# mhsitu/welding_robot

Measured on AMD Instinct MI355X. Metric: acs_generations_per_sec, higher is better.
Workload: dtype f32

## Files before the change

welding_robot_amd/csrc/acs_converged.hpp:

```cpp
#pragma once

#define WA_CONV_CHECK_WAVES 4
#define WA_CONV_ADV_WAVES 4
#define WA_CONV_THREADS ((WA_CONV_CHECK_WAVES + WA_CONV_ADV_WAVES) * 64)
#define WA_CONV_BLOCKS 64
#define WA_CONV_BLOCKS_MAX 256
#define WA_CONV_MAX_WINDOW 64
#define WA_CONV_NODE_CAP 1024
#define WA_CONV_NODE_LDS 128
#define WA_CONV_SNAP 14

struct WaConvHdr {
    uint32_t rem;
    uint32_t ticket;
    int32_t pending;
    int32_t carried;
    unsigned long long whole, cut, gens;
    int32_t end;
    int32_t pad1_;
    unsigned long long walks;
    unsigned long long pad2_;
};
static_assert(WA_CONV_SNAP == 14, "wa_table_rows strides the owed records by 14 floats");
static_assert(sizeof(WaConvHdr) == 64, "the snapshots start 64 bytes into the block");

__device__ __forceinline__ WaConvHdr *wa_conv_hdr(const WaAcsDev &D, int32_t slot) { return reinterpret_cast<WaConvHdr *>(D.conv + (int64_t)slot * D.conv_stride); }
__device__ __forceinline__ float *wa_conv_snap(const WaAcsDev &D, int32_t slot, int32_t t)
{
    return reinterpret_cast<float *>(D.conv + (int64_t)slot * D.conv_stride + sizeof(WaConvHdr)) + (int64_t)t * D.conv_nodes * WA_CONV_SNAP;
}
__device__ __forceinline__ int32_t wa_conv_pending(const WaAcsDev &D, int32_t slot) { return wa_conv_hdr(D, slot)->pending; }
__device__ __forceinline__ bool wa_conv_carried(const WaAcsDev &D, int32_t slot) { return wa_conv_hdr(D, slot)->carried != 0; }
__device__ __forceinline__ bool wa_conv_carried_at(const WaAcsDev &D, int32_t slot, int32_t gen)
{
    if (!D.conv) return false;
    const WaConvHdr *h = wa_conv_hdr(D, slot);
    return h->carried != 0 && h->end == gen && D.ctl[slot].spec_until == gen;
}
__device__ __forceinline__ void wa_conv_count_walk(const WaAcsDev &D, int32_t slot) { wa_conv_hdr(D, slot)->walks += 1; }
__device__ __forceinline__ const float *wa_conv_owed_records(const WaAcsDev &D, int32_t slot) { return wa_conv_snap(D, slot, wa_conv_pending(D, slot) - 1); }
#define WA_CONV_CARRIED 0x80u

__device__ __forceinline__ void wa_conv_flush_rows(const WaAcsDev &D, int32_t slot, int32_t first, int32_t step, bool rows_only)
{
    const int32_t blen = D.ctl[slot].best_len, j = wa_conv_pending(D, slot);
    if (j < 1) return;
    const float *snap = wa_conv_snap(D, slot, j - 1);
    const int32_t *bpath = D.bestpath + (int64_t)slot * D.path_cap;
    float *pher = D.pher + (int64_t)slot * D.pher_stride;
    float *T = D.rtab + (int64_t)slot * D.path_cap * 8;
    for (int32_t x = first; x < blen * WA_CONV_SNAP; x += step) {
        const int32_t i = x / WA_CONV_SNAP, q = x - i * WA_CONV_SNAP;
        const float v = snap[x];
        if (q < 6) { if (!rows_only) pher[(int64_t)(bpath[i] & (int32_t)WA_ID_MASK) * 6 + q] = v; }
        else T[(int64_t)i * 8 + (q - 6)] = v;
    }
}

__device__ __forceinline__ void wa_conv_ctl_step(WaSlotCtl &c, const WaRun &R, int32_t gen)
{
    const int32_t lane = threadIdx.x & 63, o = lane + 1;
    const int32_t colony = c.colony[gen & 1];
    const float lambda = c.lambda[gen & 1], Q = c.Q[gen & 1], bestL = c.bestL;
    const bool ok = lane < colony && !(bestL == INFINITY || (float)o > lambda - 1);
    const unsigned long long dep = __ballot(ok);
    const int32_t n_dep = dep ? 64 - (int32_t)__clzll((long long)dep) : 0;
    if (lane == 0) {
        c.dep_lambda = lambda;
        c.dep_Q = Q;
        c.dep_bestL = bestL;
        c.n_dep = n_dep;
        c.gen = gen + 1;
        c.rep_mask = n_dep >= 64 ? ~0ULL : (1ULL << n_dep) - 1ULL;
        c.clean[(gen + 1) & 1] = c.clean[gen & 1] * R.rho;
        wa_next_params(c, R, (gen + 1) & 1);
    }
}

__device__ __forceinline__ void wa_conv_report(uint32_t *verdict, int32_t slot, uint32_t seq, int32_t j, bool carried = false)
{
    if (!verdict) return;
    if (j > 0) {
        __threadfence_system();
        __hip_atomic_store(verdict + slot, (seq << 8) | (carried ? WA_CONV_CARRIED : 0u) | (uint32_t)j, __ATOMIC_RELEASE, __HIP_MEMORY_SCOPE_SYSTEM);
    } else __hip_atomic_store(verdict + slot, seq << 8, __ATOMIC_RELAXED, __HIP_MEMORY_SCOPE_SYSTEM);
}

__device__ __forceinline__ float wa_add_all_ranked(float p, bool on, float dep_lane, float bonus, int32_t n)
{
    n = __builtin_amdgcn_readfirstlane(n);
    const float t_lane = (int32_t)(threadIdx.x & 63) < n ? dep_lane + bonus : -0.f;
    float q = p;
    asm volatile("" : "+v"(q));
#pragma unroll
    for (int b0 = 0; b0 < 64; b0 += 8) {
        if (b0 >= n) break;
        float t[8];
#pragma unroll
        for (int j = 0; j < 8; j++) t[j] = __int_as_float(__builtin_amdgcn_readlane(__float_as_int(t_lane), b0 + j));
#pragma unroll
        for (int j = 0; j < 8; j++) q = q + t[j];
    }
    return on ? q : p;
}

__host__ __device__ inline int32_t wa_conv_share(int32_t nodes, int32_t blocks) { return (nodes + blocks - 1) / blocks; }

struct WaConvShared {
    WaSlotCtl tab[WA_CONV_MAX_WINDOW + 1];
    unsigned long long key[WA_CONV_MAX_WINDOW + 1];
    int32_t bad[WA_CONV_MAX_WINDOW + 1];
    int32_t run;
    int32_t last, j, carried;
};
__host__ __device__ inline size_t wa_conv_lds_bytes(int32_t conv_nodes, int32_t blocks)
{
    return (size_t)wa_conv_share(conv_nodes, blocks) * WA_CONV_NODE_LDS + sizeof(WaConvShared);
}

__global__ __launch_bounds__(WA_CONV_THREADS) void k_converged_run(WaAcsDev D, WaRun R, int32_t gen0, int32_t W, uint32_t *verdict, uint32_t seq, int32_t judge)
{
    extern __shared__ __attribute__((aligned(16))) float wa_conv_lds[];
    const int32_t slot = blockIdx.y, blk = blockIdx.x, nblk = gridDim.x, tid = threadIdx.x, lane = tid & 63, wave = tid >> 6;
    WaSlotCtl *ctl = &D.ctl[slot];
    WaConvHdr *hdr = wa_conv_hdr(D, slot);
    const float bestL = ctl->bestL;
    const int32_t blen = ctl->best_len;
    bool off = bestL == INFINITY || blen < 2 || blen > D.conv_nodes || blen > WA_CONV_NODE_CAP || W < 1 || W > WA_CONV_MAX_WINDOW;
    if (D.pool_n) {
        const WaStrag sg = wa_strag_of(D, slot);
        off = off || sg.pool_n[0] != 0 || sg.pool_n[1] != 0;
    }
    if (off) {
        if (blk == 0 && tid == 0) wa_conv_report(verdict, slot, seq, 0);
        return;
    }
    const int32_t cap = wa_conv_share(D.conv_nodes, nblk);
    const int32_t m = wa_conv_share(blen, nblk), n0 = blk * m;
    const int32_t mine = blen - n0 < 0 ? 0 : blen - n0 < m ? blen - n0 : m;
    const int32_t last = blen - 1;
    const int32_t ndec = (n0 + mine < last ? n0 + mine : last) - n0;
    float *s_row = wa_conv_lds;
    float *s_rec = wa_conv_lds + cap * 16;
    WaConvShared &S = *reinterpret_cast<WaConvShared *>(wa_conv_lds + cap * 32);
    {
        const int32_t *bpath = D.bestpath + (int64_t)slot * D.path_cap + n0;
        const uint8_t *btabu = D.besttabu + (int64_t)slot * D.path_cap + n0;
        const float *pher = D.pher + (int64_t)slot * D.pher_stride;
        const float *heur = D.heur + (int64_t)ctl->heur_slot * D.pher_stride;
        const float *T = D.rtab + ((int64_t)slot * D.path_cap + n0) * 8;
        for (int32_t x = tid; x < mine * 16; x += WA_CONV_THREADS) {
            const int32_t i = x >> 4, q = x & 15;
            const int64_t v = bpath[i] & (int32_t)WA_ID_MASK;
            s_rec[x] = q < 6 ? pher[v * 6 + q] : q < 12 ? heur[v * 6 + q - 6] : q == 12 ? __uint_as_float((uint32_t)btabu[i]) : 0.f;
        }
        for (int32_t x = tid; x < mine * 8; x += WA_CONV_THREADS) {
            const float v = T[x];
            s_row[x] = v;
            if ((x & 7) == 7) s_row[cap * 8 + x] = v;
        }
    }
    if (wave == 0) {
        if (lane == 0) S.tab[0] = *ctl;
        int32_t run = 0;
        for (; run < W; run++) {
            const int32_t gen = gen0 + run;
            const int32_t colony = S.tab[run].colony[gen & 1];
            if (!(colony >= 1 && colony <= D.max_colony)) break;
            if (lane == 0) S.tab[run + 1] = S.tab[run];
            wa_conv_ctl_step(S.tab[run + 1], R, gen);
        }
        if (lane == 0) S.run = run;
    } else if (wave == 1) {
        for (int32_t t = lane; t <= W; t += 64) {
            S.key[t] = wa_ctr_key(R.seed, ctl->stream, (uint32_t)(gen0 + t));
            S.bad[t] = 0;
        }
    }
    __syncthreads();
    const int32_t run = S.run;
    int32_t my_t = mine > 0 ? run : W;
    for (int32_t t = 0; t < run && mine > 0; t++) {
        const int32_t gen = gen0 + t;
        const int32_t colony = S.tab[t].colony[gen & 1];
        const float *row = s_row + (t & 1) * cap * 8;
        if (wave < WA_CONV_CHECK_WAVES) {
            const uint64_t genkey = S.key[t];
            for (int32_t a = tid; a < colony; a += WA_CONV_CHECK_WAVES * 64) {
                const uint64_t antkey = wa_ctr_antkey(genkey, (uint32_t)a);
                bool bad = false;
                for (int32_t n = 0; n < ndec; n++) {
                    const float4 *r4 = reinterpret_cast<const float4 *>(row + n * 8);
                    const float4 ca = r4[0], cb = r4[1];
                    const uint32_t h = wa_replay_hits(ca, cb, (int32_t)wa_ctr_draw(antkey, (uint32_t)(n0 + n)));
                    const int pick = h ? 31 - __clz((int)h) : -1;
                    bad = bad || pick != __float_as_int(cb.w);
                }
                if (bad) S.bad[t] = 1;
            }
        } else {
            const WaSlotCtl &c = S.tab[t + 1];
            const int32_t n_dep = c.n_dep;
            const float lambda = c.dep_lambda, Q = c.dep_Q;
            const bool okl = lane < colony && lane < n_dep;
            const float dep_lane = okl ? (lambda - (float)(lane + 1)) * Q / bestL : 0.f;
            const float bonus_on = wa_uniform(1.f * lambda * Q / bestL);
            float *nrow = s_row + ((t + 1) & 1) * cap * 8;
            float *snap = wa_conv_snap(D, slot, t) + (int64_t)n0 * WA_CONV_SNAP;
            const int32_t k2 = lane & 15, kk = k2 < 6 ? k2 : 5;
            for (int32_t i = (wave - WA_CONV_CHECK_WAVES) * 4 + (lane >> 4); __any(i < mine); i += WA_CONV_ADV_WAVES * 4) {
                const bool live = i < mine;
                const int32_t ii = live ? i : 0;
                const int32_t nk = __float_as_int(row[ii * 8 + 7]);
                float p = s_rec[ii * 16 + kk] * R.rho;
                const float h = s_rec[ii * 16 + 6 + kk];
                const uint32_t bt = __float_as_uint(s_rec[ii * 16 + 12]);
                p = wa_add_all_ranked(p, live && k2 == nk, dep_lane, bonus_on, n_dep);
                float thr, tot;
                wa_row_values(R, p, h, k2, bt, thr, tot);
                if (!live) continue;
                float *sn = snap + i * WA_CONV_SNAP;
                if (k2 < 6) {
                    s_rec[i * 16 + k2] = p;
                    nrow[i * 8 + k2] = thr;
                    sn[k2] = p;
                    sn[6 + k2] = thr;
                }
                if (k2 == 5) { nrow[i * 8 + 6] = tot; sn[12] = tot; }
                if (k2 == 0) sn[13] = __int_as_float(nk);
            }
        }
        __syncthreads();
        if (S.bad[t] != 0) { my_t = t; break; }
    }
    int32_t leaves = 1;
    if (judge && run == W && my_t == W) {
        const int32_t gen = gen0 + W;
        const int32_t colony = S.tab[W].colony[gen & 1];
        leaves = !(colony >= 1 && colony <= D.max_colony);
        if (!leaves && mine > 0) {
            if (wave < WA_CONV_CHECK_WAVES) {
                const float *row = s_row + (W & 1) * cap * 8;
                const uint64_t genkey = S.key[W];
                for (int32_t a = tid; a < colony; a += WA_CONV_CHECK_WAVES * 64) {
                    const uint64_t antkey = wa_ctr_antkey(genkey, (uint32_t)a);
                    bool bad = false;
                    for (int32_t n = 0; n < ndec; n++) {
                        const float4 *r4 = reinterpret_cast<const float4 *>(row + n * 8);
                        const float4 ca = r4[0], cb = r4[1];
                        const uint32_t h = wa_replay_hits(ca, cb, (int32_t)wa_ctr_draw(antkey, (uint32_t)(n0 + n)));
                        const int pick = h ? 31 - __clz((int)h) : -1;
                        bad = bad || pick != __float_as_int(cb.w);
                    }
                    if (bad) S.bad[W] = 1;
                }
            }
            __syncthreads();
            leaves = S.bad[W] != 0;
        }
    }
    if (tid == 0) {
        atomicMax(&hdr->rem, ((uint32_t)(W - my_t) << 1) | (uint32_t)leaves);
        __threadfence();
        const uint32_t tk = atomicAdd(&hdr->ticket, 1u);
        int32_t is_last = 0, j = 0, carried = 0;
        if (tk == (uint32_t)nblk - 1u) {
            __threadfence();
            is_last = 1;
            const uint32_t rem = atomicMax(&hdr->rem, 0u);
            j = W - (int32_t)(rem >> 1);
            carried = rem == 0u;
        }
        S.last = is_last;
        S.j = j;
        S.carried = carried;
    }
    __syncthreads();
    if (!S.last) return;
    const int32_t j = S.j;
    const bool carried = S.carried != 0;
    if (tid == 0) {
        hdr->rem = 0;
        hdr->ticket = 0;
        if (j > 0) {
            WaSlotCtl c = S.tab[j];
            c.spec_until = gen0 + j;
            *ctl = c;
            hdr->pending = j;
            hdr->carried = carried ? 1 : 0;
            hdr->end = gen0 + j;
            hdr->gens += (unsigned long long)j;
            if (j == W) hdr->whole += 1; else hdr->cut += 1;
        }
    }
    if (j > 0) {
        const int32_t colony = S.tab[j].colony[(gen0 + j - 1) & 1];
        const float lambda = S.tab[j].dep_lambda, Q = S.tab[j].dep_Q;
        for (int32_t r = tid; r < colony; r += WA_CONV_THREADS) {
            const int32_t o = r + 1;
            const bool ok = !(bestL == INFINITY || (float)o > lambda - 1);
            D.perm[(int64_t)slot * D.max_colony + r] = r;
            D.depA[(int64_t)slot * D.max_colony + r] = ok ? (lambda - (float)o) * Q / bestL : 0.f;
        }
        for (int32_t t = tid; t < j; t += WA_CONV_THREADS) {
            const int32_t gen = gen0 + t;
            if (gen >= D.trace_cap) continue;
            const int32_t col = S.tab[t].colony[gen & 1];
            const int64_t tr = (int64_t)slot * D.trace_cap + gen;
            D.trBest[tr] = bestL;
            D.trIter[tr] = bestL;
            D.trColony[tr] = col;
            D.trFinite[tr] = col;
            D.trSteps[tr] = (long long)col * (long long)(blen - 1);
        }
    }
    __syncthreads();
    if (tid == 0) wa_conv_report(verdict, slot, seq, j, carried);
}
```

welding_robot_amd/csrc/host_acs.inc:

```
static int acs_drain(wa_acs *s);
void wa_acs_default_params(wa_acs_params *p)
{
    if (!p) return;
    p->alpha = 1;
    p->beta = 0.6f;
    p->rho = 0.8f;
    p->pheromone_0 = 1.f;
    p->max_iteration = 150;
    p->predict = 10.f;
    p->fixed_colony = 0;
    p->rng_mode = WA_RNG_DEV;
    p->seed = 1;
}


static_assert(WA_PLAN_REF_SPEC_LEN == WA_REF_SPEC_LEN && WA_PLAN_REF_SUPER == WA_REF_SUPER && WA_PLAN_RESUME_MAX == WA_RESUME_MAX &&
              WA_PLAN_POOL_REC == WA_POOL_REC && WA_PLAN_ROW26 == WA_ROW26, "acs_plan.hpp and the kernels' headers disagree");
static WaPlanIn acs_plan_in(const wa_grid *grid, int32_t n_slots, int32_t max_colony, int64_t path_capacity, int32_t nb, bool lazy)
{
    int32_t fields0 = n_slots < 4 ? n_slots : 4;
    if (n_slots >= 32) fields0 = n_slots / 8 < 8 ? 8 : (n_slots / 8 > 24 ? 24 : n_slots / 8);
    return WaPlanIn{grid->d.n, grid->d.nxy, n_slots, max_colony, fields0, path_capacity, nb, lazy ? 1 : 0,
                    env_int("WA_MASK_U64", 0), env_int("WA_REPLAY", 1), env_int("WA_REF_SPEC", 1), env_int("WA_STRAGGLERS", 1), env_int("WA_STRAGGLER_SLOTS", 16),
                    (int64_t)sizeof(WaSlotCtl), (int64_t)sizeof(WaGlibcRand)};
// ... 40 lines not shown
    s->nb = nb;
    s->lazy = lazy;
    s->slot_buf.assign(n_slots, 0);
    s->lazy_mode.assign(n_slots, -1);
    s->lazy_p0.assign(n_slots, 0.f);
    if (nb == 6 && 24 * n >= (int64_t)1 << 31) {
        delete s;
        return fail(ctx, WA_ERR_ARG, "wa_acs_create: grids above 89,478,485 voxels (~447^3) are not supported");
    }
    if (nb == 26 && n > (int64_t)WaNbT<26>::IDM + 1) {
        delete s;
        return fail(ctx, WA_ERR_ARG, "wa_acs_create: 26-neighbour grids above 2^27 voxels (512^3) are not supported");
    }
    const WaAcsPlan &P = s->plan = wa_acs_plan(acs_plan_in(grid, n_slots, max_colony, path_capacity, nb, lazy));
    path_capacity = s->path_cap = P.cap;
    s->ref_spec = P.ref_spec;
    WaAcsDev &D = s->D;
    D.d = grid->d;
    D.cx = grid->cx; D.cy = grid->cy; D.cz = grid->cz; D.occ = grid->occ;
    D.nb = nb;
    D.max_colony = max_colony;
    D.pher_stride = P.pher_stride; D.path_cap = P.cap; D.vbits_words = P.vbits_words; D.vbits_rows = (int32_t)P.vbits_rows;
    D.guard_bytes = (int32_t)(P.guard * sizeof(float)); D.stamp_guard_bytes = (int32_t)(P.sguard * sizeof(uint32_t));
    int lg = 11;
    while ((1 << lg) < 64 * (grid->d.nx + grid->d.ny + grid->d.nz) && lg < 15) lg++;
    int id_bits = 1;
    while (((int64_t)1 << id_bits) < n) id_bits++;
    s->tab16_env = env_int("WA_TAB16", -1);
    s->id_bits = id_bits;
    D.tab16_kmul = 0;
    if (nb == 6 && id_bits <= 27 && s->tab16_env != 0) {
        uint32_t kb = (uint32_t)((double)((uint64_t)1 << id_bits) * 0.6180339887498949) | 1u;
        D.tab16_kmul = kb << (32 - id_bits);
    }
    {
        const int64_t blocks = (int64_t)n_slots * max_colony;
        const bool saturated = blocks > ctx->prop.multiProcessorCount;
        auto capacity = [&](int l) {
            const bool t16 = saturated && D.tab16_kmul != 0 && id_bits <= l + 12 && (s->tab16_env == 1 || id_bits <= 21);
            int64_t per_cu = 160 * 1024 / (((t16 ? 2 : 4) << l) + WA_WALK_LDS_EXTRA);
            if (per_cu > 16) per_cu = 16;
            return per_cu * ctx->prop.multiProcessorCount;
        };
        int floor_lg = 6;
        while (floor_lg < 15 && 3 * ((int64_t)1 << floor_lg) < 16 * (int64_t)(grid->d.nx + grid->d.ny + grid->d.nz)) floor_lg++;
        if (floor_lg < 10) floor_lg = 10;
        while (lg > floor_lg && capacity(lg) < blocks && capacity(lg - 1) > capacity(lg)) lg--;
        if (n_slots == 1 && !lazy && max_colony <= 256 && env_int("WA_STRAGGLERS", 1))
            while (lg > 12 && capacity(lg) < max_colony + WA_RESUME_MAX) lg--;
    }
    s->hash_log2 = env_int("WA_HASH_LOG2", lg);
    if (s->hash_log2 < 6) s->hash_log2 = 6;
    if (s->hash_log2 > 15) s->hash_log2 = 15;
    s->walk_asm = env_int("WA_WALK_ASM", 1) != 0;
    s->walk_warm = env_int("WA_WALK_WARM", -1);
    s->walk_direct = env_int("WA_WALK_DIRECT", -1);
    s->lds_pad = env_int("WA_WALK_LDS_PAD", 0);
    if (s->lds_pad < 0 || (sizeof(int32_t) << s->hash_log2) + (size_t)s->lds_pad > (sizeof(int32_t) << 15)) s->lds_pad = 0;
    {
        const int re = env_int("WA_REENTRY", 1);
        s->walk_flags = (s->walk_asm ? 1 : 0) | (re ? 2 : 0) | ((env_int("WA_REENTRY_STABLE", 16) & 127) << 24);
#ifdef WA_TEST_KNOBS
        s->walk_flags |= (re == 2 ? 4 : 0) | (env_int("WA_REENTRY_ANYWHERE", 0) ? 8 : 0) | ((env_int("WA_REENTRY_HOLD", 0) & 0xffff) << 8);
#endif
    }
    s->lazy_blocks_env = env_int("WA_LAZY_BLOCKS", 0);
    s->pipe_groups_env = env_int("WA_PIPE_GROUPS", 0);
    s->hw_queues = env_int("GPU_MAX_HW_QUEUES", 4);
    s->drain_ok = env_int("WA_STRAGGLER_DRAIN", 1) != 0;
    s->sweep_nt_env = env_int("WA_SWEEP_NT", -1);
    s->straggler_gens = env_int("WA_STRAGGLER_GENS", 64);
    s->conv_on = env_int("WA_CONVERGED_RUN", 1) != 0;
    s->conv_window = env_int("WA_CONVERGED_WINDOW", 32);
    if (s->conv_window > WA_CONV_MAX_WINDOW) s->conv_window = WA_CONV_MAX_WINDOW;
    if (s->conv_window < 1) s->conv_on = false;
    s->conv_nodes_env = env_int("WA_CONVERGED_NODES", 0);
    s->conv_blocks = env_int("WA_CONVERGED_BLOCKS", WA_CONV_BLOCKS);
    s->conv_blocks = s->conv_blocks < 1 ? 1 : s->conv_blocks > WA_CONV_BLOCKS_MAX ? WA_CONV_BLOCKS_MAX : s->conv_blocks;
    s->conv_readback = env_int("WA_CONVERGED_READBACK", 1) != 0;
    s->conv_wait_us = env_int("WA_CONVERGED_WAIT_US", 200000);
    s->conv_spec = env_int("WA_CONVERGED_SPECULATE", 1) != 0;
    s->conv_owed = env_int("WA_CONVERGED_OWED", 1) != 0;
    s->conv_cwalk = env_int("WA_CONVERGED_CARRIED_WALK", 1) != 0;
    s->prof_dispatch = env_int("WA_PROF_DISPATCH", 1) != 0;
    s->conv_enqueued.assign((size_t)n_slots, 0);
    {
        const int64_t n4 = (int64_t)nb * n / 4;
        int64_t blocks = n4 <= ((int64_t)8 << 20) ? 4096 : n4 / 555;
        if (blocks > 65536) blocks = 65536;
        s->evap_blocks = env_int("WA_EVAP_BLOCKS", (int)blocks);
    }
    hipError_t e = hipSuccess;
    const bool trace_create = env_int("WA_TRACE_CREATE", 0) != 0;
    const auto t_create0 = std::chrono::steady_clock::now();
    auto since0 = [&]() { return std::chrono::duration<double>(std::chrono::steady_clock::now() - t_create0).count(); };
    bool pools = P.pools;
    for (const WaPlanRow &r : P.rows) {
        if (e || (r.pool && !pools)) continue;
        if (&r == &P.rows[P.heur_row]) { e = (hipError_t)heur_pool_grow(s, &D, (int32_t)P.fields0); continue; }
        void *p = nullptr;
        const hipError_t re = ctx_alloc_bytes(ctx, &p, (size_t)P.bytes(r));
        if (re == hipSuccess) { s->blocks.push_back(WaBlock{&r, p}); continue; }
        if (!r.pool) { e = re; continue; }
        (void)hipGetLastError();
        pools = false;
        for (; s->blocks.back().row->pool; s->blocks.pop_back()) ctx_free(ctx, s->blocks.back().p);
    }
    size_t wired = 0;
    auto wire = [&](auto *&dst, const char *name, int64_t skip = 0) {
        using T = typename std::remove_reference<decltype(dst)>::type;
        for (const WaBlock &b : s->blocks)
            if (!strcmp(b.row->name, name)) { dst = static_cast<T>(b.p) + skip; wired++; }
    };
    uint32_t *ref_jump = nullptr;
    wire(s->pher_buf[0], "pher0", P.guard); wire(s->pher_buf[1], "pher1", P.guard); wire(D.heur, "heur", P.guard); wire(D.ltab, "ltab");
    wire(D.stamp, "stamp", P.sguard); wire(D.dirty_list, "dirty_list"); wire(D.dcount, "dcount");
    wire(D.mask8, "mask8"); wire(D.mask, "mask"); wire(D.bestmark, "bestmark"); wire(D.bestpath, "bestpath"); wire(D.bestpos, "bestpos"); wire(D.besttabu, "besttabu"); wire(D.rtab, "rtab");
    wire(D.paths, "paths"); wire(D.antL, "antL"); wire(D.antLen, "antLen"); wire(D.perm, "perm"); wire(D.depA, "depA"); wire(D.sortk, "sortk");
    wire(D.vbits, "vbits"); wire(D.ctl, "ctl"); wire(D.rng, "rng"); wire(D.dbg, "dbg");
    wire(D.ref_draws, "ref_draws"); wire(D.ref_state, "ref_state"); wire(D.ref_ok, "ref_ok"); wire(ref_jump, "ref_jump");
    s->paths_arr[0] = s->paths_arr[1] = D.paths;
    wire(s->paths_arr[1], "paths2"); wire(D.arr_len, "arr_len"); wire(D.arr_n, "arr_n"); wire(D.pool_rec, "pool_rec"); wire(D.pool_n, "pool_n"); wire(D.strag_cnt, "strag_cnt");
    wire(s->d_starts, "d_starts"); wire(s->d_ends, "d_ends"); wire(s->d_streams, "d_streams"); wire(s->d_hslot, "d_hslot"); wire(s->d_hlist, "d_hlist"); wire(s->d_hends, "d_hends");
    if (D.antLen) D.antRep = D.antLen + (size_t)n_slots * max_colony;
    D.ref_jump = ref_jump;
    D.pher = s->pher_buf[0];
    if (!e && wired != s->blocks.size()) e = hipErrorInvalidValue;
    if (e != hipSuccess) {
        wa_acs_destroy(s);
        return fail(ctx, WA_ERR_ALLOC, "wa_acs_create: device allocation failed: %s", hipGetErrorString(e));
    }
    const double t_alloc = since0();
    for (const WaBlock &b : s->blocks) {
        if (b.row->fill == WA_FILL_NONE) continue;
        const size_t bytes = (size_t)P.bytes(*b.row), skip = b.row->upper_half ? bytes / 2 : 0;
        e = e ? e : hipMemsetAsync((char *)b.p + skip, b.row->fill == WA_FILL_ONES ? 0xff : 0, bytes - skip, ctx->stream);
    }
    if (P.ref_spec) {
        static std::vector<uint32_t> J;
        if (J.empty()) {
            auto mul = [](const std::vector<uint32_t> &A, const std::vector<uint32_t> &B) {
                std::vector<uint32_t> Cm(31 * 31, 0u);
                for (int i = 0; i < 31; i++)
                    for (int k = 0; k < 31; k++) {
                        const uint32_t a = A[i * 31 + k];
                        if (a) for (int j = 0; j < 31; j++) Cm[i * 31 + j] += a * B[k * 31 + j];
                    }
                return Cm;
            };
            std::vector<uint32_t> Pm(31 * 31, 0u), Rm(31 * 31, 0u);
            for (int j = 0; j < 30; j++) Pm[j * 31 + j + 1] = 1u;
            Pm[30 * 31 + 0] = 1u; Pm[30 * 31 + 28] = 1u;
            for (int i = 0; i < 31; i++) Rm[i * 31 + i] = 1u;
            for (int k = WA_REF_SUPER; k; k >>= 1) { if (k & 1) Rm = mul(Rm, Pm); Pm = mul(Pm, Pm); }
            J = Rm;
        }
        e = e ? e : hipMemcpyAsync(ref_jump, J.data(), sizeof(uint32_t) * 31 * 31, hipMemcpyHostToDevice, ctx->stream);
    }
    {
        std::vector<float> &lt = s->ltab_host;
        lt.assign((size_t)path_capacity + 1, 0.f);
        float L = 0.f;
        for (size_t i = 0; i < lt.size(); i++) { lt[i] = L; L += grid->precision; }
        e = e ? e : hipMemcpyAsync(D.ltab, lt.data(), sizeof(float) * lt.size(), hipMemcpyHostToDevice, ctx->stream);
    }
    WaGlibcRand r0;
// ... 555 lines not shown
            const int32_t SLd = G.P >= 32 ? 1 : 2, TBd = G.P >= 32 ? 32 : WA_TABLE_BLOCKS_MAX;
            if (s->nb == 26) hipExtLaunchKernelGGL(k_apply_table26, dim3((unsigned)(1 + WA_TABLE26_BLOCKS + mark_blocks(s)), (unsigned)P), dim3(256), 0, st, dp.a, dp.b, 0, G.V, s->R);
            else hipExtLaunchKernelGGL(k_apply_table, dim3((unsigned)(TBd + ((mark_blocks(s) >> 3) << SLd)), (unsigned)P), dim3(256), 0, st, dp.a, dp.b, 0, G.V, s->R, SLd, TBd, owed ? gen | WA_GEN_OWED : gen);
            s->ev.push_back(dp);
        }
        else if (s->nb == 26) k_apply_table26<<<dim3((unsigned)(1 + WA_TABLE26_BLOCKS + mark_blocks(s)), (unsigned)P), 256, 0, st>>>(G.V, s->R);
        else { const int32_t SL = P >= 32 ? 1 : 2, TB = P >= 32 ? 32 : WA_TABLE_BLOCKS_MAX; k_apply_table<<<dim3((unsigned)(TB + ((mark_blocks(s) >> 3) << SL)), (unsigned)P), 256, 0, st>>>(G.V, s->R, SL, TB, owed ? gen | WA_GEN_OWED : gen); }
        prof_close(st, e);
        WA_DBG_SYNC("apply+table");
        WA_HASH_AT(2);
        return;
    }
    e = prof_open(s, st, WA_K_RANK, sampled);
    if (s->nb == 26) k_rank<26><<<P, 256, 0, st>>>(G.V, s->R, gen);
    else k_rank<6><<<P, 256, 0, st>>>(G.V, s->R, gen);
    prof_close(st, e);
    launch_evaporate(s, st, s->pher_buf[G.cur], s->pher_buf[G.cur ^ 1], G.slot0, P, s->R.rho, sampled, G.sweep_nt);
    G.cur ^= 1;
    G.V.pher = dst;
    e = prof_open(s, st, WA_K_DEPOSIT, sampled);
    for (int32_t c = 0; c < chunks; c++) {
        dim3 dg(8, 64, (unsigned)P);
        if (s->nb == 26) {
            k_deposit_mark<26><<<dg, 256, 0, st>>>(G.V, c * 64);
            k_deposit_apply<26><<<dg, 256, 0, st>>>(G.V, c * 64);
        } else {
            k_deposit_mark<6><<<dg, 256, 0, st>>>(G.V, c * 64);
            k_deposit_apply<6><<<dg, 256, 0, st>>>(G.V, c * 64);
        }
    }
    if (s->D.rtab && (s->R.rng_mode == WA_RNG_DEV || (s->ref_spec && s->nb == 6 && s->R.alpha == 1))) {
        if (s->nb == 26) k_replay_table26<<<dim3(257, (unsigned)P), 64, 0, st>>>(G.V, s->R);
        else k_replay_table<<<dim3(32, (unsigned)P), 256, 0, st>>>(G.V, s->R);
    }
    prof_close(st, e);
}

static bool conv_rule(const wa_acs *s, bool fused)
{
#ifdef WA_STATE_HASH
    return false;
#endif
    return s->conv_on && fused && !s->lazy && s->nb == 6 && s->R.rng_mode == WA_RNG_DEV && s->D.rtab != nullptr && s->colony_bound > 0;
}
static bool conv_scratch(wa_acs *s)
{
    if (s->d_conv && s->conv_snaps >= s->conv_window) return true;
    wa_ctx *ctx = s->ctx;
    if (s->conv_readback && !s->h_verdict) {
        void *w = nullptr;
        if (hipHostMalloc(&w, sizeof(uint32_t) * (size_t)s->n_slots, hipHostMallocCoherent) != hipSuccess) { (void)hipGetLastError(); s->conv_readback = false; }
        else { memset(w, 0, sizeof(uint32_t) * (size_t)s->n_slots); s->h_verdict = static_cast<uint32_t *>(w); }
    }
    if (s->d_conv) { hipStreamSynchronize(ctx->stream); ctx_free(ctx, s->d_conv); s->d_conv = nullptr; s->D.conv = nullptr; }
    int64_t nodes = s->D.path_cap < WA_CONV_NODE_CAP ? s->D.path_cap : WA_CONV_NODE_CAP;
    if (s->conv_nodes_env > 0 && s->conv_nodes_env < nodes) nodes = s->conv_nodes_env;
    const int64_t stride = (int64_t)sizeof(WaConvHdr) + (int64_t)s->conv_window * nodes * WA_CONV_SNAP * (int64_t)sizeof(float);
    void *blk = nullptr;
    if (ctx_alloc_bytes(ctx, &blk, (size_t)(stride * s->n_slots)) != hipSuccess) { (void)hipGetLastError(); s->conv_on = false; return false; }
    if (hipMemsetAsync(blk, 0, (size_t)(stride * s->n_slots), ctx->stream) != hipSuccess) { ctx_free(ctx, blk); s->conv_on = false; return false; }
    s->d_conv = static_cast<char *>(blk);
    s->conv_snaps = s->conv_window;
    s->D.conv = s->d_conv;
    s->D.conv_stride = stride;
    s->D.conv_nodes = (int32_t)nodes;
    return true;
}
static int32_t conv_window_at(const wa_acs *s, int32_t gen, int32_t gen_last)
{
    int32_t W = s->conv_window;
    if (gen_last - gen < W) W = gen_last - gen;
    if (s->prof_sweep_all) return 0;
    if (s->prof) {
        if (gen % s->prof_every == 0) return 0;
        const int32_t next = (gen / s->prof_every + 1) * s->prof_every;
        if (next - gen < W) W = next - gen;
    }
    return W < 0 ? 0 : W;
}
static hipError_t launch_converged(wa_acs *s, WaGroupRun &G, int32_t gen, int32_t W, bool judge)
{
    G.V.pher = s->pher_buf[G.cur] + (int64_t)G.slot0 * s->D.pher_stride;
    uint32_t *verdict = s->conv_readback && s->h_verdict ? s->h_verdict + G.slot0 : nullptr;
    k_converged_run<<<dim3((unsigned)s->conv_blocks, (unsigned)G.P), WA_CONV_THREADS, wa_conv_lds_bytes(s->D.conv_nodes, s->conv_blocks), G.st>>>(
        G.V, s->R, gen, W, verdict, s->conv_seq & 0xffffffu, judge ? 1 : 0);
    for (int32_t q = 0; q < G.P; q++) s->conv_enqueued[(size_t)(G.slot0 + q)]++;
    return hipGetLastError();
}
#define WA_CONV_QUERY_US 2000
static int32_t conv_verdict(wa_acs *s, hipStream_t st, int32_t W)
{
    const uint32_t want = s->conv_seq & 0xffffffu;
    const uint32_t *word = s->h_verdict;
    s->conv_host[0]++;
    int32_t j = -1;
    uint32_t got = 0;
    s->conv_carried = false;
    if (s->conv_wait_us > 0) {
        const auto t0 = std::chrono::steady_clock::now();
        int64_t next_query = WA_CONV_QUERY_US;
        for (uint32_t spin = 1;; spin++) {
            uint32_t v = __atomic_load_n(word, __ATOMIC_ACQUIRE);
            if ((v >> 8) == want) { got = v; j = (int32_t)(v & 0x7fu); break; }
            if (spin & 255u) { __builtin_ia32_pause(); continue; }
            const int64_t waited = std::chrono::duration_cast<std::chrono::microseconds>(std::chrono::steady_clock::now() - t0).count();
            if (waited > s->conv_wait_us) break;
            if (waited >= next_query) {
                next_query = waited + WA_CONV_QUERY_US;
                const hipError_t q = hipStreamQuery(st);
                if (q == hipErrorNotReady) { (void)hipGetLastError(); continue; }
                v = __atomic_load_n(word, __ATOMIC_ACQUIRE);
                if ((v >> 8) == want) { got = v; j = (int32_t)(v & 0x7fu); }
                break;
            }
        }
    }
    if (j < 0 || j > W) { s->conv_host[3]++; return -1; }
    s->conv_carried = j == W && (got & WA_CONV_CARRIED) != 0;
    return j;
}

static int acs_drain(wa_acs *s)
{
    s->read_since_run = true;
    if (!s->pending_resume) return WA_OK;
    s->pending_resume = false;
    wa_ctx *ctx = s->ctx;
    if (!s->begun || !s->D.pool_n || s->gens_enqueued < 1) return WA_OK;
    const int32_t P = s->n_active, gen = s->gens_enqueued;
    const size_t shmem = (sizeof(int32_t) << s->hash_log2) + WA_WALK_LDS_EXTRA + (size_t)s->lds_pad;
    WaAcsDev V = s->D;
    V.pher = s->pher_buf[s->cur_buf];
    V.prev_pher = s->pher_buf[s->cur_buf ^ 1];
    V.paths = s->paths_arr[gen & 1];
    V.prev_paths = s->paths_arr[(gen + 1) & 1];
    dim3 wg((unsigned)(s->D.max_colony + WA_RESUME_MAX), (unsigned)P);
    const int walk_flags = (s->walk_flags & 1) | 64;
    if (s->nb == 26) k_walk_dev26<false><<<wg, 64, shmem, ctx->stream>>>(V, s->R, s->hash_log2, gen, walk_flags);
    else k_walk_dev<true, false, true, false><<<wg, 64, shmem, ctx->stream>>>(V, s->R, s->hash_log2, gen, walk_flags);
    HIPC(ctx, hipGetLastError());
    HIPC(ctx, hipMemset2DAsync(s->D.pool_n + ((gen - 1) & 1), sizeof(int32_t) * 2, 0, sizeof(int32_t), (size_t)P, ctx->stream));
    return WA_OK;
}

static int32_t pipe_groups(const wa_acs *s, int32_t P)
{
    int32_t g = s->pipe_groups_env > 0 ? s->pipe_groups_env : (P >= (s->lazy ? 4 : 2) ? 2 : 1);
    if (s->pipe_groups_env <= 0 && s->lazy && P >= 6 && s->colony_bound >= 128) g = 3;
    if (s->pipe_groups_env <= 0 && g > s->hw_queues) g = s->hw_queues;
    if (s->R.rng_mode != WA_RNG_DEV) g = 1;
    if (g > P) g = P;
    return g < 1 ? 1 : g;
}

int wa_acs_set_pipeline(wa_acs *s, int32_t groups)
{
    if (!s || groups < 0) return WA_ERR_ARG;
    s->pipe_groups_env = groups;
    return WA_OK;
}
int wa_acs_walk_info(const wa_acs *s, int32_t out[4])
{
    if (!s || !out) return WA_ERR_ARG;
    for (int i = 0; i < 4; i++) out[i] = s->last_walk[i];
    return WA_OK;
}
int wa_acs_pipeline_info(const wa_acs *s, int32_t *groups_last_run)
{
    if (!s) return WA_ERR_ARG;
    if (groups_last_run) *groups_last_run = s->last_groups;
    return WA_OK;
}

static hipError_t enqueue_spec_flush(wa_acs *s, WaGroupRun &G, int32_t gen, int32_t gflags)
{
    const int64_t off = (int64_t)G.slot0 * s->D.pher_stride;
    float *src = s->pher_buf[G.cur] + off, *dst = s->pher_buf[G.cur ^ 1] + off;
    G.V.pher = src;
    G.V.prev_pher = dst;
    launch_fused(s, G, src, dst, gen | gflags, false);
    G.cur ^= 1;
    G.V.pher = dst;
    const int32_t SL = 2, TB = WA_TABLE_BLOCKS_MAX;
    k_apply_table<<<dim3((unsigned)(TB + ((mark_blocks(s) >> 3) << SL)), (unsigned)G.P), 256, 0, G.st>>>(G.V, s->R, SL, TB, gen | gflags);
    return hipGetLastError();
}
static hipError_t enqueue_owed_rows(wa_acs *s, WaGroupRun &G, int32_t gen)
{
    G.cur ^= 1;
    G.V.pher = s->pher_buf[G.cur] + (int64_t)G.slot0 * s->D.pher_stride;
    const int32_t SL = 2, TB = WA_TABLE_BLOCKS_MAX;
    k_apply_table<<<dim3((unsigned)TB, (unsigned)G.P), 256, 0, G.st>>>(G.V, s->R, SL, TB, gen | WA_GEN_OWED);
    return hipGetLastError();
}

int wa_acs_run(wa_acs *s, int32_t n_generations)
{
    WaDevGuard dev_guard_(s ? s->ctx : nullptr);
    if (!dev_guard_.ok) return WA_ERR_DEVICE;
    if (!s || n_generations < 0) return WA_ERR_ARG;
    wa_ctx *ctx = s->ctx;
    if (!s->begun) return fail(ctx, WA_ERR_STATE, "wa_acs_run before wa_acs_begin");
    const int32_t P = s->n_active;
    const size_t shmem = (sizeof(int32_t) << s->hash_log2) + WA_WALK_LDS_EXTRA + (size_t)s->lds_pad;
    if (!ctx->lds_attr_set) {
        const int lds_max = (int)((sizeof(int32_t) << 15) + WA_WALK_LDS_EXTRA);
        hipError_t a = hipSuccess;
#define WA_LDS_ATTR(...) a = a ? a : hipFuncSetAttribute((const void *)k_walk_dev<__VA_ARGS__>, hipFuncAttributeMaxDynamicSharedMemorySize, lds_max)
        WA_LDS_ATTR(false, false, true, true); WA_LDS_ATTR(false, true, true, true);
        WA_LDS_ATTR(true, false, true, true); WA_LDS_ATTR(true, false, true, false); WA_LDS_ATTR(true, false, false, true); WA_LDS_ATTR(true, false, false, false);
        WA_LDS_ATTR(true, true, true, true); WA_LDS_ATTR(true, true, true, false); WA_LDS_ATTR(true, true, false, true); WA_LDS_ATTR(true, true, false, false);
        WA_LDS_ATTR(true, false, false, true, true); WA_LDS_ATTR(true, false, false, false, true); WA_LDS_ATTR(true, true, false, true, true); WA_LDS_ATTR(true, true, false, false, true);
        WA_LDS_ATTR(true, false, false, true, false, true); WA_LDS_ATTR(true, false, false, false, false, true); WA_LDS_ATTR(true, true, false, true, false, true); WA_LDS_ATTR(true, true, false, false, false, true);
#undef WA_LDS_ATTR
        a = a ? a : hipFuncSetAttribute((const void *)k_converged_run, hipFuncAttributeMaxDynamicSharedMemorySize, (int)wa_conv_lds_bytes(WA_CONV_NODE_CAP, 1));
        a = a ? a : hipFuncSetAttribute((const void *)k_walk_ref, hipFuncAttributeMaxDynamicSharedMemorySize, lds_max);
        a = a ? a : hipFuncSetAttribute((const void *)k_walk_dev26<false>, hipFuncAttributeMaxDynamicSharedMemorySize, lds_max);
        a = a ? a : hipFuncSetAttribute((const void *)k_walk_dev26<true>, hipFuncAttributeMaxDynamicSharedMemorySize, lds_max);
        a = a ? a : hipFuncSetAttribute((const void *)k_walk_ref26, hipFuncAttributeMaxDynamicSharedMemorySize, lds_max);
        if (a != hipSuccess) return fail(ctx, WA_ERR_DEVICE, "wa_acs_run: dynamic LDS limit of the walk kernels: %s", hipGetErrorString(a));
        ctx->lds_attr_set = true;
    }
    const int32_t dep_bound = (int32_t)(0.2 * s->colony_bound) + 1;
    const int32_t chunks = (dep_bound + 63) / 64;
    const bool fused = s->lazy || (s->R.rng_mode == WA_RNG_DEV && s->colony_bound <= WA_RANK_LDS && dep_bound <= 64 && s->D.rtab);
    if (n_generations > 0) {
        s->res_valid = false;
        s->chained = s->ran_before && !s->read_since_run;
        s->ran_before = true;
        s->read_since_run = false;
    }
    if (n_generations > 0 && s->pending_resume) {
        const bool carries = s->D.pool_n != nullptr && fused && s->R.rng_mode == WA_RNG_DEV && s->R.alpha == 1 && s->gens_enqueued <= s->straggler_gens;
        if (carries) s->pending_resume = false;
        else { int drc_ = acs_drain(s); if (drc_) return drc_; }
    }
#ifdef WA_STATE_HASH
    if (n_generations > 0 && s->gens_enqueued == 0) {
        const size_t bytes = sizeof(unsigned long long) * 256 * 3 * (size_t)s->n_slots * 8;
        if (!s->d_hashlog) HIPC(ctx, dev_malloc((void **)&s->d_hashlog, bytes));
        HIPC(ctx, hipMemsetAsync(s->d_hashlog, 0, bytes, ctx->stream));
    }
#endif
    const bool conv = n_generations > 1 && conv_rule(s, fused) && conv_scratch(s);
    const bool readback = conv && s->conv_readback && s->h_verdict && P == 1;
    const bool owed_on = readback && s->conv_owed;
    const bool cwalk = owed_on && s->conv_cwalk;
    const int32_t gen_last = s->gens_enqueued + n_generations - 1;
    const int32_t NG = n_generations > 0 ? pipe_groups(s, P) : 1;
    s->last_groups = NG;
    std::vector<WaGroupRun> groups((size_t)NG);
    if (NG > 1) {
        while ((int32_t)s->gstream.size() < NG - 1) {
            hipStream_t st = nullptr;
            hipEvent_t ev = nullptr;
            HIPC(ctx, hipStreamCreateWithFlags(&st, hipStreamNonBlocking));
            s->gstream.push_back(st);
            HIPC(ctx, hipEventCreateWithFlags(&ev, hipEventDisableTiming));
            s->gjoin.push_back(ev);
        }
        if (!s->gfork) HIPC(ctx, hipEventCreateWithFlags(&s->gfork, hipEventDisableTiming));
        HIPC(ctx, hipEventRecord(s->gfork, ctx->stream));
    }
    for (int32_t k = 0; k < NG; k++) {
        WaGroupRun &G = groups[(size_t)k];
        G.slot0 = (int32_t)((int64_t)P * k / NG);
        G.P = (int32_t)((int64_t)P * (k + 1) / NG) - G.slot0;
        G.st = k > 0 ? s->gstream[(size_t)k - 1] : ctx->stream;
        G.V = dev_view(s, G.slot0);
        G.cur = s->cur_buf;
        G.sweep_nt = sweep_policy(s, P);
        if (k > 0) HIPC(ctx, hipStreamWaitEvent(G.st, s->gfork, 0));
    }
    for (int32_t g = 0; g < n_generations; g++) {
        const bool sampled = s->prof && ((s->gens_enqueued % s->prof_every) == 0);
        const int32_t gen = s->gens_enqueued;
        int32_t ask = 0;
        bool owe = false;
        if (gen == s->conv_owed_flush) {
            s->conv_owed_flush = -1;
            if (cwalk) {
                groups[0].cur ^= 1;
                s->conv_cwalk_info[1]++;
            } else {
                const hipError_t re = enqueue_owed_rows(s, groups[0], gen);
                if (re != hipSuccess) return fail(ctx, WA_ERR_DEVICE, "wa_acs_run: rows of a carried window: %s", hipGetErrorString(re));
            }
            s->conv_owed_gen = gen + 1;
            s->gens_enqueued++;
            continue;
        }
        const bool owed = gen == s->conv_owed_gen;
        if (owed) {
            s->conv_owed_gen = -1;
            s->conv_owed_info[1]++;
            s->conv_owed_info[(s->conv_owed_reps & 1) ? 3 : 4]++;
        }
        if (conv && gen >= s->conv_until) {
// ... 518 lines not shown
```

welding_robot_amd/csrc/weldacs.hip:

```cpp
#include "../../include/weldacs.h"

#include <hip/hip_runtime.h>
#include <hip/hip_ext.h>
#include <rccl/rccl.h>

#include <float.h>
#include <locale.h>
#include <math.h>
#include <stdio.h>
#include <stdlib.h>
#include <string.h>

#include <algorithm>
#include <atomic>
#include <chrono>
#include <functional>
#include <memory>
#include <mutex>
#include <thread>
#include <unordered_map>
#include <string>
#include <vector>

#include "acs_kernels.hpp"
// ... 89 lines not shown
    const wa_grid *grid = nullptr;
    int32_t n_slots = 0, max_colony = 0, n_active = 0, nb = 6;
    int64_t path_cap = 0;
    WaAcsDev D = {};
    WaAcsPlan plan;
    std::vector<WaBlock> blocks;
    int32_t *d_stage = nullptr;
    size_t stage_words = 0;
    std::vector<float> ltab_host;
    std::vector<WaSlotCtl> res_ctl;
    std::vector<int32_t> res_words;
    int64_t res_longest = 0;
    bool res_valid = false;
    int32_t *paths_arr[2] = {nullptr, nullptr};
    float *pher_buf[2] = {nullptr, nullptr};
    int cur_buf = 0;
    std::vector<int> slot_buf;
    bool walk_asm = true;
    int walk_warm = -1;
    int32_t last_walk[4] = {0, 0, 0, 0};
#ifdef WA_STATE_HASH
    unsigned long long *d_hashlog = nullptr;
#endif
    int tab16_env = -1, id_bits = 0;
    int lds_pad = 0;
    int walk_direct = -1;
    int walk_flags = 0;
    WaRun R = {};
    bool begun = false;
    bool lazy = false;
    std::vector<int> lazy_mode;
    std::vector<float> lazy_p0;
    int32_t gens_enqueued = 0, colony_bound = 0, hash_log2 = 0, evap_blocks = 0, lazy_blocks_env = 0, straggler_gens = 64;
    long long *d_starts = nullptr, *d_ends = nullptr;
    uint32_t *d_streams = nullptr;
    int32_t *d_hslot = nullptr, *d_hlist = nullptr, *d_hends = nullptr;
    int32_t heur_fields = 0;
    std::vector<long long> heur_end;
    std::vector<float> heur_beta;
    std::vector<long long> heur_used;
    long long heur_batch = 0;
    bool prof = false, prof_sweep_all = false;
    bool prof_paired = false;
    int32_t prof_every = 1;
    std::vector<EvPair> ev;
    std::vector<EvPair> ev_pool;
    bool prof_dispatch = true;
    double prof_ms[WA_K_COUNT] = {};
    int64_t prof_n[WA_K_COUNT] = {};
    int32_t pipe_groups_env = 0;
    int32_t hw_queues = 4;
    std::vector<hipStream_t> gstream;
    std::vector<hipEvent_t> gjoin;
    int32_t sweep_nt_env = -1;
    hipEvent_t gfork = nullptr;
    int32_t last_groups = 1;
    bool ref_spec = true;
    bool drain_ok = true;
    bool pending_resume = false;
    bool ran_before = false, read_since_run = false, chained = false;
    bool conv_on = true;
    int32_t conv_window = 32;
    int32_t conv_blocks = 0;
    int32_t conv_nodes_env = 0;
    int32_t conv_until = 0;
    char *d_conv = nullptr;
    int32_t conv_snaps = 0;
    std::vector<uint64_t> conv_enqueued;
    bool conv_readback = true;
    int32_t conv_wait_us = 200000;
    uint32_t *h_verdict = nullptr;
    uint32_t conv_seq = 0;
    uint64_t conv_host[4] = {0, 0, 0, 0};
    bool conv_spec = true;
    bool conv_owed = true;
    bool conv_carried = false;
    int32_t conv_owed_flush = -1;
    int32_t conv_owed_gen = -1;
    int32_t conv_owed_reps = 0;
    uint64_t conv_owed_info[5] = {0, 0, 0, 0, 0};
    bool conv_cwalk = true;
    int32_t conv_walk_done = -1;
    uint64_t conv_cwalk_info[4] = {0, 0, 0, 0};
    bool conv_prev_whole = false;
};

static int fail(wa_ctx *c, int code, const char *fmt, const char *a = "", const char *b = "")
{
    if (c) {
        char buf[512];
        snprintf(buf, sizeof buf, fmt, a, b);
        c->err = buf;
    }
    return code;
}
#define HIPC(ctx, call)                                                                       \
    do {                                                                                      \
        hipError_t e_ = (call);                                                               \
        if (e_ != hipSuccess) return fail((ctx), WA_ERR_DEVICE, #call ": %s", hipGetErrorString(e_)); \
    } while (0)

static thread_local const wa_ctx *g_alloc_ctx = nullptr;
struct WaDevGuard {
    int prev = -1;
    bool switched = false, ok = true, named = false;
    const wa_ctx *prev_named = nullptr;
    explicit WaDevGuard(const wa_ctx *c)
    {
        if (!c) return;
        prev_named = g_alloc_ctx;
        g_alloc_ctx = (c->poison || c->guard) ? c : nullptr;
        named = true;
        if (hipGetDevice(&prev) != hipSuccess) prev = -1;
        if (prev != c->device) {
            ok = hipSetDevice(c->device) == hipSuccess;
            switched = ok && prev >= 0;
        }
    }
    ~WaDevGuard()
    {
        if (named) g_alloc_ctx = prev_named;
        if (switched) hipSetDevice(prev);
    }
    WaDevGuard(const WaDevGuard &) = delete;
    WaDevGuard &operator=(const WaDevGuard &) = delete;
};

static int env_int(const char *name, int def)
{
    const char *v = getenv(name);
    return v && *v ? atoi(v) : def;
}

static std::mutex g_cache_mu;
static std::vector<wa_ctx *> g_cache_ctxs;
static const size_t WA_CACHE_MIN_BYTES = (size_t)1 << 20;
static const size_t WA_ARENA_SZ[3] = {(size_t)512 << 20, (size_t)32 << 20, (size_t)2 << 20}, WA_ARENA_MIN = (size_t)2 << 20;
enum { WA_ST_ALLOCS = 0, WA_ST_HIT_BYTES, WA_ST_MISS_BYTES, WA_ST_RELEASED_BYTES, WA_ST_FULL_HITS, WA_ST_OOM_EVENTS, WA_ST_WAIT_MS };

static hipMemAllocationProp arena_prop(int device)
{
    hipMemAllocationProp prop = {};
    prop.type = hipMemAllocationTypePinned;
    prop.location.type = hipMemLocationTypeDevice;
    prop.location.id = device;
    return prop;
}

static const uintptr_t WA_VA_FIRST = (uintptr_t)32 << 40, WA_VA_END = (uintptr_t)96 << 40;
static uintptr_t g_va_cursor = WA_VA_FIRST, g_va_end = WA_VA_END;
static bool g_va_exhausted = false;
static bool g_va_nohint = false;
static hipError_t va_reserve_fresh_locked(size_t bytes, void **out)
{
    *out = nullptr;
    if (g_va_exhausted) return hipErrorOutOfMemory;
    const uintptr_t align = bytes >= WA_ARENA_SZ[0] ? (uintptr_t)1 << 30 : bytes >= WA_ARENA_SZ[1] ? (uintptr_t)WA_ARENA_SZ[1] : (uintptr_t)WA_ARENA_SZ[2];
    for (int tries = 0; tries < 8; tries++) {
        const uintptr_t start = (g_va_cursor + align - 1) & ~(align - 1);
        if (start + bytes > g_va_end || start + bytes < start) { g_va_exhausted = true; return hipErrorOutOfMemory; }
        void *hint = (void *)start, *va = nullptr;
        const hipError_t e = hipMemAddressReserve(&va, bytes, 0, g_va_nohint ? nullptr : hint, 0);
        if (e != hipSuccess) { (void)hipGetLastError(); g_va_cursor = start + ((uintptr_t)1 << 40); continue; }
        if (va == hint) {
            g_va_cursor = start + bytes + (uintptr_t)WA_ARENA_SZ[2];
            *out = va;
// ... 626 lines not shown
```

Measured before the change: 34440.

## Overlap the converged-run control chain with replay checks using a dedicated wave

Adds a templated variant of the converged-run kernel with a ninth wave. That wave computes each generation's control record one step ahead while the check and advance waves process the current generation. Before, wave 0 walked the whole control chain serially before any checking started, so that prologue is now hidden behind the per-generation work. The extra wave raises block size and per-generation barrier participation, and the run length is now found lazily inside the loop. The variant is on by default via an environment variable.

```diff
diff --git a/welding_robot_amd/csrc/acs_converged.hpp b/welding_robot_amd/csrc/acs_converged.hpp
--- a/welding_robot_amd/csrc/acs_converged.hpp
+++ b/welding_robot_amd/csrc/acs_converged.hpp
@@ -3,6 +3,8 @@
 #define WA_CONV_CHECK_WAVES 4
 #define WA_CONV_ADV_WAVES 4
 #define WA_CONV_THREADS ((WA_CONV_CHECK_WAVES + WA_CONV_ADV_WAVES) * 64)
+#define WA_CONV_CHAIN_WAVE (WA_CONV_CHECK_WAVES + WA_CONV_ADV_WAVES)
+#define WA_CONV_THREADS_CHAIN (WA_CONV_THREADS + 64)
 #define WA_CONV_BLOCKS 64
 #define WA_CONV_BLOCKS_MAX 256
 #define WA_CONV_MAX_WINDOW 64
@@ -118,9 +120,21 @@
     return (size_t)wa_conv_share(conv_nodes, blocks) * WA_CONV_NODE_LDS + sizeof(WaConvShared);
 }
 
-__global__ __launch_bounds__(WA_CONV_THREADS) void k_converged_run(WaAcsDev D, WaRun R, int32_t gen0, int32_t W, uint32_t *verdict, uint32_t seq, int32_t judge)
+__device__ __forceinline__ bool wa_conv_chain_step(WaConvShared &S, const WaAcsDev &D, const WaRun &R, int32_t gen0, int32_t u)
+{
+    const int32_t gen = gen0 + u;
+    const int32_t colony = S.tab[u].colony[gen & 1];
+    if (!(colony >= 1 && colony <= D.max_colony)) return false;
+    if ((threadIdx.x & 63) == 0) S.tab[u + 1] = S.tab[u];
+    wa_conv_ctl_step(S.tab[u + 1], R, gen);
+    return true;
+}
+
+template <bool CHAIN_AHEAD>
+__global__ __launch_bounds__(CHAIN_AHEAD ? WA_CONV_THREADS_CHAIN : WA_CONV_THREADS) void k_converged_run(WaAcsDev D, WaRun R, int32_t gen0, int32_t W, uint32_t *verdict, uint32_t seq, int32_t judge)
 {
     extern __shared__ __attribute__((aligned(16))) float wa_conv_lds[];
+    constexpr int32_t NT = CHAIN_AHEAD ? WA_CONV_THREADS_CHAIN : WA_CONV_THREADS;
     const int32_t slot = blockIdx.y, blk = blockIdx.x, nblk = gridDim.x, tid = threadIdx.x, lane = tid & 63, wave = tid >> 6;
     WaSlotCtl *ctl = &D.ctl[slot];
     WaConvHdr *hdr = wa_conv_hdr(D, slot);
@@ -149,18 +163,28 @@
         const float *pher = D.pher + (int64_t)slot * D.pher_stride;
         const float *heur = D.heur + (int64_t)ctl->heur_slot * D.pher_stride;
         const float *T = D.rtab + ((int64_t)slot * D.path_cap + n0) * 8;
-        for (int32_t x = tid; x < mine * 16; x += WA_CONV_THREADS) {
+        for (int32_t x = tid; x < mine * 16; x += NT) {
             const int32_t i = x >> 4, q = x & 15;
             const int64_t v = bpath[i] & (int32_t)WA_ID_MASK;
             s_rec[x] = q < 6 ? pher[v * 6 + q] : q < 12 ? heur[v * 6 + q - 6] : q == 12 ? __uint_as_float((uint32_t)btabu[i]) : 0.f;
         }
-        for (int32_t x = tid; x < mine * 8; x += WA_CONV_THREADS) {
+        for (int32_t x = tid; x < mine * 8; x += NT) {
             const float v = T[x];
             s_row[x] = v;
             if ((x & 7) == 7) s_row[cap * 8 + x] = v;
         }
     }
-    if (wave == 0) {
+    if (CHAIN_AHEAD) {
+        if (wave == WA_CONV_CHAIN_WAVE) {
+            if (lane == 0) S.tab[0] = *ctl;
+            wa_conv_chain_step(S, D, R, gen0, 0);
+        } else if (wave == 1) {
+            for (int32_t t = lane; t <= W; t += 64) {
+                S.key[t] = wa_ctr_key(R.seed, ctl->stream, (uint32_t)(gen0 + t));
+                S.bad[t] = 0;
+            }
+        }
+    } else if (wave == 0) {
         if (lane == 0) S.tab[0] = *ctl;
         int32_t run = 0;
         for (; run < W; run++) {
@@ -178,13 +202,17 @@
         }
     }
     __syncthreads();
-    const int32_t run = S.run;
-    int32_t my_t = mine > 0 ? run : W;
-    for (int32_t t = 0; t < run && mine > 0; t++) {
+    int32_t run = CHAIN_AHEAD ? W : S.run;
+    int32_t my_t = -1;
+    for (int32_t t = 0; t < run && (CHAIN_AHEAD || mine > 0); t++) {
         const int32_t gen = gen0 + t;
         const int32_t colony = S.tab[t].colony[gen & 1];
+        if (CHAIN_AHEAD && !(colony >= 1 && colony <= D.max_colony)) { run = t; break; }
         const float *row = s_row + (t & 1) * cap * 8;
-        if (wave < WA_CONV_CHECK_WAVES) {
+        if (CHAIN_AHEAD && wave == WA_CONV_CHAIN_WAVE) {
+            if (t + 1 < W) wa_conv_chain_step(S, D, R, gen0, t + 1);
+        } else if (mine <= 0) {
+        } else if (wave < WA_CONV_CHECK_WAVES) {
             const uint64_t genkey = S.key[t];
             for (int32_t a = tid; a < colony; a += WA_CONV_CHECK_WAVES * 64) {
                 const uint64_t antkey = wa_ctr_antkey(genkey, (uint32_t)a);
@@ -233,6 +261,7 @@
         __syncthreads();
         if (S.bad[t] != 0) { my_t = t; break; }
     }
+    if (my_t < 0) my_t = mine > 0 ? run : W;
     int32_t leaves = 1;
     if (judge && run == W && my_t == W) {
         const int32_t gen = gen0 + W;
@@ -296,13 +325,13 @@
     if (j > 0) {
         const int32_t colony = S.tab[j].colony[(gen0 + j - 1) & 1];
         const float lambda = S.tab[j].dep_lambda, Q = S.tab[j].dep_Q;
-        for (int32_t r = tid; r < colony; r += WA_CONV_THREADS) {
+        for (int32_t r = tid; r < colony; r += NT) {
             const int32_t o = r + 1;
             const bool ok = !(bestL == INFINITY || (float)o > lambda - 1);
             D.perm[(int64_t)slot * D.max_colony + r] = r;
             D.depA[(int64_t)slot * D.max_colony + r] = ok ? (lambda - (float)o) * Q / bestL : 0.f;
         }
-        for (int32_t t = tid; t < j; t += WA_CONV_THREADS) {
+        for (int32_t t = tid; t < j; t += NT) {
             const int32_t gen = gen0 + t;
             if (gen >= D.trace_cap) continue;
             const int32_t col = S.tab[t].colony[gen & 1];
diff --git a/welding_robot_amd/csrc/host_acs.inc b/welding_robot_amd/csrc/host_acs.inc
--- a/welding_robot_amd/csrc/host_acs.inc
+++ b/welding_robot_amd/csrc/host_acs.inc
@@ -146,6 +146,7 @@
     s->conv_spec = env_int("WA_CONVERGED_SPECULATE", 1) != 0;
     s->conv_owed = env_int("WA_CONVERGED_OWED", 1) != 0;
     s->conv_cwalk = env_int("WA_CONVERGED_CARRIED_WALK", 1) != 0;
+    s->conv_chain_ahead = env_int("WA_CONVERGED_CHAIN_AHEAD", 1) != 0;
     s->prof_dispatch = env_int("WA_PROF_DISPATCH", 1) != 0;
     s->conv_enqueued.assign((size_t)n_slots, 0);
     {
@@ -867,8 +868,10 @@
 {
     G.V.pher = s->pher_buf[G.cur] + (int64_t)G.slot0 * s->D.pher_stride;
     uint32_t *verdict = s->conv_readback && s->h_verdict ? s->h_verdict + G.slot0 : nullptr;
-    k_converged_run<<<dim3((unsigned)s->conv_blocks, (unsigned)G.P), WA_CONV_THREADS, wa_conv_lds_bytes(s->D.conv_nodes, s->conv_blocks), G.st>>>(
-        G.V, s->R, gen, W, verdict, s->conv_seq & 0xffffffu, judge ? 1 : 0);
+    const dim3 cgrid((unsigned)s->conv_blocks, (unsigned)G.P);
+    const size_t clds = wa_conv_lds_bytes(s->D.conv_nodes, s->conv_blocks);
+    if (s->conv_chain_ahead) k_converged_run<true><<<cgrid, WA_CONV_THREADS_CHAIN, clds, G.st>>>(G.V, s->R, gen, W, verdict, s->conv_seq & 0xffffffu, judge ? 1 : 0);
+    else k_converged_run<false><<<cgrid, WA_CONV_THREADS, clds, G.st>>>(G.V, s->R, gen, W, verdict, s->conv_seq & 0xffffffu, judge ? 1 : 0);
     for (int32_t q = 0; q < G.P; q++) s->conv_enqueued[(size_t)(G.slot0 + q)]++;
     return hipGetLastError();
 }
@@ -998,7 +1001,8 @@
         WA_LDS_ATTR(true, false, false, true, true); WA_LDS_ATTR(true, false, false, false, true); WA_LDS_ATTR(true, true, false, true, true); WA_LDS_ATTR(true, true, false, false, true);
         WA_LDS_ATTR(true, false, false, true, false, true); WA_LDS_ATTR(true, false, false, false, false, true); WA_LDS_ATTR(true, true, false, true, false, true); WA_LDS_ATTR(true, true, false, false, false, true);
 #undef WA_LDS_ATTR
-        a = a ? a : hipFuncSetAttribute((const void *)k_converged_run, hipFuncAttributeMaxDynamicSharedMemorySize, (int)wa_conv_lds_bytes(WA_CONV_NODE_CAP, 1));
+        a = a ? a : hipFuncSetAttribute((const void *)k_converged_run<false>, hipFuncAttributeMaxDynamicSharedMemorySize, (int)wa_conv_lds_bytes(WA_CONV_NODE_CAP, 1));
+        a = a ? a : hipFuncSetAttribute((const void *)k_converged_run<true>, hipFuncAttributeMaxDynamicSharedMemorySize, (int)wa_conv_lds_bytes(WA_CONV_NODE_CAP, 1));
         a = a ? a : hipFuncSetAttribute((const void *)k_walk_ref, hipFuncAttributeMaxDynamicSharedMemorySize, lds_max);
         a = a ? a : hipFuncSetAttribute((const void *)k_walk_dev26<false>, hipFuncAttributeMaxDynamicSharedMemorySize, lds_max);
         a = a ? a : hipFuncSetAttribute((const void *)k_walk_dev26<true>, hipFuncAttributeMaxDynamicSharedMemorySize, lds_max);
diff --git a/welding_robot_amd/csrc/weldacs.hip b/welding_robot_amd/csrc/weldacs.hip
--- a/welding_robot_amd/csrc/weldacs.hip
+++ b/welding_robot_amd/csrc/weldacs.hip
@@ -195,6 +195,7 @@
     bool conv_cwalk = true;
     int32_t conv_walk_done = -1;
     uint64_t conv_cwalk_info[4] = {0, 0, 0, 0};
+    bool conv_chain_ahead = true;
     bool conv_prev_whole = false;
 };
 
```

After: 34720, median of 6. Within noise of the previous version (+0.8%).
